# Oliverbansk/Holistic-Robot-Pose-Estimation

Measured on AMD Instinct MI355X. Metric: images/sec/GPU fwd+bwd HRNet-W32 256x256 bs=64; 1/2/4/8-GPU scaling, higher is better.
Workload: dtype bf16; 1 GPU; full network (HRNet-W32 reg backbone + HRNet-W32 DepthNet + heads + FK loss) fwd+loss+bwd+clip+Adam, BASELINE.json configs[2]; global_batch=64, per_gpu_batch=64, image=3x256x256, hrnet_w32_passes_per_image=2, parallelism=dp1, backend=single-process, rccl_ranks=1, hip_graph=True, plan_mode=hybrid, inputs=resident in HBM, optimizer=hrpe_amd.optim.FusedClipAdam (clip 5 + Adam, lr 1e-4)

## Files before the change

### holistic-robot-pose-estimation_amd/_native.py

```python
import ctypes as C
import os
import subprocess

_HERE = os.path.dirname(os.path.abspath(__file__))
LIB_PATH = os.environ.get("HRP_LIB") or os.path.join(_HERE, "libhrp_hip.so")
CSRC = os.path.join(_HERE, "csrc")

HRP_F32, HRP_BF16, HRP_F32X3 = 0, 1, 2
MAX_TAPS = 16
EW_MAX_IN = 4
EW_IDENTITY, EW_AFFINE, EW_BN_TRAIN = 0, 1, 2
FK_MAX_JOINTS, FK_MAX_KP = 32, 24
PIL_KMAX = 12


class HrpError(RuntimeError):
    pass


class ConvDesc(C.Structure):
    _fields_ = [("x", C.c_void_p), ("w", C.c_void_p), ("y", C.c_void_p), ("res", C.c_void_p),
                ("bias", C.c_void_p), ("scale", C.c_void_p), ("shift", C.c_void_p), ("stats", C.c_void_p),
                ("dtype", C.c_int32),
                ("N", C.c_int32), ("H", C.c_int32), ("W", C.c_int32), ("Cin", C.c_int32), ("x_pitch", C.c_int32),
# ... 130 lines not shown
class OptChunk(C.Structure):
    _fields_ = [("tensor", C.c_int32), ("offset", C.c_int32)]


class RegStepDesc(C.Structure):
    _fields_ = [("M", C.c_int32), ("P", C.c_int32), ("K", C.c_int32), ("N", C.c_int32),
                ("u_prev", C.c_void_p), ("u_bias", C.c_void_p), ("z", C.c_void_p), ("zw", C.c_void_p),
                ("z_len", C.c_int32), ("z_pitch", C.c_int32), ("zw_sk", C.c_int32), ("zw_sp", C.c_int32),
                ("u_out", C.c_void_p), ("a", C.c_void_p), ("a_mask", C.c_void_p), ("v", C.c_void_p),
                ("a_pitch", C.c_int32), ("v_sk", C.c_int32), ("v_sp", C.c_int32), ("a2_pitch", C.c_int32),
                ("a_out", C.c_void_p), ("w", C.c_void_p), ("bias", C.c_void_p), ("out_mask", C.c_void_p),
                ("a2", C.c_void_p), ("w2", C.c_void_p), ("w_sn", C.c_int64), ("w_sk", C.c_int64),
                ("out_pitch", C.c_int32), ("out_accumulate", C.c_int32), ("out_sum_accumulate", C.c_int32), ("w2_sk", C.c_int32),
                ("out", C.c_void_p), ("out_sum", C.c_void_p)]


class LinWgradDesc(C.Structure):
    _fields_ = [("x", C.c_void_p), ("dy", C.c_void_p), ("dw", C.c_void_p), ("dbias", C.c_void_p),
                ("x_pitch", C.c_int32), ("dy_pitch", C.c_int32), ("dw_ld", C.c_int32), ("M", C.c_int32),
                ("K", C.c_int32), ("N", C.c_int32), ("accumulate", C.c_int32), ("reserved", C.c_int32)]


REG_MAX_P, REG_MAX_PROBLEMS, LIN_WGRAD_MAX = 16, 4, 8
COPY_MAX = 16


class CopyDesc(C.Structure):
    _fields_ = [("src", C.c_void_p), ("dst", C.c_void_p), ("src_pitch", C.c_int), ("dst_pitch", C.c_int), ("rows", C.c_int),
                ("cols", C.c_int), ("accumulate", C.c_int), ("reserved", C.c_int)]


def copy_cols_batch(items, stream):
    for i0 in range(0, len(items), COPY_MAX):
        grp = items[i0:i0 + COPY_MAX]
        arr = (CopyDesc * len(grp))()
        for d, (src, sp, dst, dp, rows, cols, acc) in zip(arr, grp):
            d.src, d.src_pitch, d.dst, d.dst_pitch, d.rows, d.cols, d.accumulate = src, sp, dst, dp, rows, cols, acc
        call("hrp_copy_cols_batch", arr, len(grp), stream)


class FkChain(C.Structure):
    _fields_ = [("njoints", C.c_int32), ("parent", C.c_int32 * FK_MAX_JOINTS), ("type", C.c_int32 * FK_MAX_JOINTS),
                ("cfg", C.c_int32 * FK_MAX_JOINTS), ("mimic_mul", C.c_float * FK_MAX_JOINTS),
                ("mimic_off", C.c_float * FK_MAX_JOINTS), ("origin", (C.c_float * 12) * FK_MAX_JOINTS),
                ("axis", (C.c_float * 3) * FK_MAX_JOINTS), ("nkp", C.c_int32), ("kp_frame", C.c_int32 * FK_MAX_KP),
                ("kp_offset", (C.c_float * 3) * FK_MAX_KP), ("dof", C.c_int32)]


DREAM_BANDS = 32
DREAM_JITTER, DREAM_OCCLUSION, DREAM_SHARPNESS, DREAM_CONTRAST, DREAM_BRIGHTNESS, DREAM_COLOR = 1, 2, 4, 8, 16, 32


class DreamSample(C.Structure):
    _fields_ = [("jitter", C.c_double * 3), ("enh", C.c_double * 4), ("flags", C.c_int32),
                ("occ_x", C.c_int32), ("occ_y", C.c_int32), ("occ_w", C.c_int32), ("occ_h", C.c_int32),
                ("pad_x", C.c_int32), ("pad_y", C.c_int32), ("work_w", C.c_int32), ("work_h", C.c_int32),
                ("crop_x0", C.c_int32), ("crop_y0", C.c_int32), ("crop_x1", C.c_int32), ("crop_y1", C.c_int32),
                ("off_x", C.c_int32), ("off_y", C.c_int32), ("side", C.c_int32), ("reserved", C.c_int32),
                ("noise_off", C.c_int64), ("scratch_off", C.c_int64)]


_P, _I, _F, _L = C.c_void_p, C.c_int, C.c_float, C.c_int64
PROTOTYPES = {
    "hrp_version": [], "hrp_device_ok": [],
    "hrp_nchw_to_nhwc": [_P, _P, _I, _I, _I, _I, _I, _I, _P],
    "hrp_nhwc_to_nchw": [_P, _P, _I, _I, _I, _I, _I, _I, _P],
    "hrp_nchw_grad_from_nhwc": [_P, _P, _I, _I, _I, _I, _I, _I, _P],
    "hrp_pack_weights": [_P, _I, _I, _I, _P],
    "hrp_pack_blocks": [_I, _I, _I, _I, _I, _I],
    "hrp_pack_weights_compact": [_P, _P, _I, _I, _I, _P],
    "hrp_nchw_to_nhwc_s2d": [_P, _P, _I, _I, _I, _I, _I, _I, _P],
    "hrp_u8_nchw_to_nhwc": [_P, _P, _I, _I, _I, _I, _I, _I, _F, _I, _P],
    "hrp_gather_f32": [_P, _P, _P, _I, _I, _P],
    "hrp_pil_resize_table": [_I, _I, _P],
    "hrp_pil_resize_normalize": [_P, _I, _I, _I, _I, _P, _P, _I, _I, _P, _I, _I, _I, _P, _P, _P],
    "hrp_broadcast_hw": [_P, _I, _P, _I, _I, _I, _I, _I, _P],
    "hrp_bilinear_nhwc_to_nchw": [_P, _I, _I, _I, _I, _I, _I, _P, _I, _I, _I, _P],
    "hrp_fill_zero": [_P, _L, _P],
    "hrp_maxpool3x3s2_fwd": [_P, _I, _I, _I, _I, _I, _I, _P, _I, _P, _P],
    "hrp_maxpool3x3s2_bwd": [_P, _I, _P, _P, _I, _I, _I, _I, _I, _I, _I, _P],
    "hrp_conv2d_fwd": [C.POINTER(ConvDesc), _P],
    "hrp_conv_rowstrip_channels": [C.POINTER(ConvDesc)],
    "hrp_conv_pointwise": [C.POINTER(ConvDesc)],
    "hrp_conv2d_bwd_weight": [C.POINTER(WgradDesc), _P],
    "hrp_colsum": [_P, _I, _L, _I, _I, _P, _I, _P, _L, _P],
    "hrp_colsum_workspace_bytes": [_L, _I],
    "hrp_ew_fwd": [C.POINTER(EwDesc), _P],
    "hrp_ew_bwd_reduce": [C.POINTER(EwBwdDesc), _P],
    "hrp_ew_pool2": [_P, _I, _I, _P, _I, _I, _I, _I, _I, _P, _P],
    "hrp_ew_bwd_apply": [C.POINTER(EwBwdDesc), _P],
    "hrp_bn_running_update": [_P, _I, _P], "hrp_bn_fold": [_P, _I, _P], "hrp_bn_param_grad": [_P, _I, _P],
    "hrp_avgpool_fwd": [_P, _I, _I, _I, _I, _I, _P, _I, _P],
    "hrp_avgpool_bwd": [_P, _I, _P, _I, _I, _I, _I, _I, _I, _P],
    "hrp_softargmax3d_fwd": [_P, _I, _I, _I, _I, _I, _I, _I, _I, _I, _P, _P, _P],
    "hrp_softargmax3d_bwd": [_P, _I, _I, _I, _I, _I, _I, _I, _I, _I, _P, _P, _P, _P, _I, _P],
    "hrp_pose_geometry_fwd": [_P, _P, _P, _P, _I, _I, _I, _F, _F, _P, _P, _P, _P, _P],
    "hrp_pose_geometry_bwd": [_P, _P, _P, _P, _I, _I, _I, _F, _F, _P, _P, _P, _P, _P, _P, _P],
    "hrp_fk_project_fwd": [_P, _P, _P, _P, _P, _I, _I, _P, _P, _P, _P],
    "hrp_fk_project_bwd": [_P, _P, _P, _P, _P, _I, _I, _P, _P, _P, _P, _P, _P],
    "hrp_fk_project_rot_fwd": [_P, _P, _P, _I, _P, _P, _I, _I, _P, _P, _P, _P],
    "hrp_fk_project_rot_bwd": [_P, _P, _P, _I, _P, _P, _I, _I, _P, _P, _P, _P, _P, _P],
    "hrp_copy_cols": [_P, _I, _P, _I, _I, _I, _I, _P],
    "hrp_copy_cols_batch": [_P, _I, _P],
    "hrp_scale_rows": [_P, _I, _I, _I, _P, _F, _P],
    "hrp_mul_f32": [_P, _I, _P, _I, _P, _I, _I, _I, _I, _P],
    "hrp_opt_grad_sumsq": [_P, _P, _I, _P, _P, _P],
    "hrp_opt_adam_step": [_P, _P, _I, _P, _F, _P, _F, _F, _F, _F, _P],
    "hrp_batch_prepare": [_I, _P, _I, _P, C.POINTER(BatchInfo)],
    "hrp_batch_launch": [_P, C.POINTER(BatchInfo), _P],
    "hrp_softargmax_flat_fwd": [_P, _I, _I, _I, _I, _I, _P, _P, _P],
    "hrp_softargmax_flat_bwd": [_P, _I, _I, _I, _I, _I, _P, _P, _P, _P, _I, _P],
    "hrp_rot6d_compose_fwd": [_P, _P, _P, _I, _P],
    "hrp_rot6d_compose_bwd": [_P, _P, _P, _P, _P, _I, _I, _I, _P],
    "hrp_wgrad_fold_desc_of": [C.POINTER(WgradDesc), C.POINTER(WgradFoldDesc)],
    "hrp_batch_wgrad_fold_descs": [_P, C.POINTER(BatchInfo), C.POINTER(WgradFoldDesc)],
    "hrp_block_channels": [C.POINTER(BlockDesc)],
    "hrp_block_prepare": [_P, _I, _P, C.POINTER(BlockInfo)],
    "hrp_block_launch": [_P, C.POINTER(BlockInfo), _P],
    "hrp_pose_loss": [C.POINTER(PoseLossDesc), _P],
    "hrp_l1_loss": [_P, _P, _F, _I, _P, _P, _P],
    "hrp_sim2real_loss": [C.POINTER(Sim2RealLossDesc), _P],
    "hrp_mesh_pose": [_P, _P, _P, _P, _I, _I, _P, _P, _I, _P, _P, _P, _P],
    "hrp_mesh_pose_bwd": [_P, _P, _P, _P, _I, _I, _P, _P, _I, _P, _P, _P, _P],
    "hrp_silhouette_fwd": [C.POINTER(SilhouetteDesc), _P],
    "hrp_silhouette_bwd": [C.POINTER(SilhouetteDesc), _P, _P, _P],
    "hrp_linear_fwd": [_P, _I, _P, _P, _P, _I, _P, _I, _I, _I, _I, _P, _L, _P],
    "hrp_linear_bwd_data": [_P, _I, _P, _P, _I, _I, _I, _I, _I, _P, _L, _P],
    "hrp_linear_workspace_bytes": [_I, _I, _I],
    "hrp_linear_bwd_weight": [_P, _I, _P, _I, _P, _P, _I, _I, _I, _I, _P],
    "hrp_rng_advance": [_P, _P],
    "hrp_dropout_f32": [_P, _I, _P, _I, _P, _I, _I, _F, _P, C.c_uint32, _P],
    "hrp_dropout_masks": [_P, _L, _F, _P, C.c_uint32, _P],
    "hrp_regressor_step": [_P, _I, _P],
    "hrp_linear_wgrad_batch": [_P, _I, _P],
    "hrp_project_fwd": [_P, _P, _I, _I, _P, _P],
    "hrp_project_bwd": [_P, _P, _P, _I, _I, _P, _P],
    "hrp_pnp_solve": [_P, _P, _I, _P, _I, _P, _I, _I, _P, _P, _P, _P],
    "hrp_pnp_bwd": [_P, _P, _I, _P, _I, _P, _P, _I, _I, _I, _P, _P, _P, _P, _P, _P, _P],
    "hrp_dream_augment": [_P, _I, _I, _I, _P, _P, _L, _I, _I, _P, _L, _P, _P],
    "hrp_dream_crop_resize": [_P, _L, _P, _P, _I, _I, _I, _P, _I, _I, _P, _I, _I, _P],
}

_lib = None


def source_hash():
    import glob
    import hashlib
    files = [os.path.basename(f) for f in glob.glob(os.path.join(CSRC, "*.hip")) + glob.glob(os.path.join(CSRC, "*.h"))]
    names = sorted(files + ["../../include/hrp.h", "Makefile"])
    h = hashlib.sha256()
    for n in names:
        with open(os.path.join(CSRC, n), "rb") as fh:
            h.update(fh.read())
    return h.hexdigest()[:16]


def build(force=False):
    if force:
        subprocess.run(["make", "-C", CSRC, "clean"], check=True, stdout=subprocess.DEVNULL)
    r = subprocess.run(["make", "-C", CSRC, "-j8"], stdout=subprocess.PIPE, stderr=subprocess.STDOUT, text=True)
    if r.returncode != 0:
        raise HrpError("building libhrp_hip.so failed:\n" + r.stdout[-4000:])
    return LIB_PATH


# ... 82 lines not shown
```

### holistic-robot-pose-estimation_amd/csrc/batch.h

```cpp
#pragma once
#include "hrp_common.h"

namespace hrp {

struct BatchHdr {
  int blk0[HRP_BATCH_MAX];
};

__device__ __forceinline__ int batch_find(const BatchHdr& h, int b, int& base) {
  int g = 0;
  base = 0;
#pragma unroll
  for (int i = 1; i < HRP_BATCH_MAX; ++i) {
    const bool ge = b >= h.blk0[i];
    g = ge ? i : g;
    base = ge ? h.blk0[i] : base;
  }
  return g;
}

static inline BatchHdr make_hdr(const int* blk0, int n) {
  BatchHdr h;
  for (int i = 0; i < HRP_BATCH_MAX; ++i) h.blk0[i] = i < n ? blk0[i] : 0x7fffffff;
  return h;
}

int conv_batch_prepare_bf16(const hrp_conv_desc* descs, int n, void* table, hrp_batch_info* info);
int conv_batch_prepare_f32(const hrp_conv_desc* descs, int n, void* table, hrp_batch_info* info);
int conv_batch_prepare_f32x3(const hrp_conv_desc* descs, int n, void* table, hrp_batch_info* info);
int conv_batch_launch_bf16(const void* table_dev, const hrp_batch_info* info, hipStream_t s);
int conv_batch_launch_f32(const void* table_dev, const hrp_batch_info* info, hipStream_t s);
int conv_batch_launch_f32x3(const void* table_dev, const hrp_batch_info* info, hipStream_t s);
int64_t conv_batch_table_bytes(int n);
int conv_check(const hrp_conv_desc* d);

int wgrad_batch_prepare(const hrp_wgrad_desc* descs, int n, void* table, hrp_batch_info* info);
int wgrad_batch_launch(const void* table_dev, const hrp_batch_info* info, hipStream_t s);
int64_t wgrad_batch_table_bytes(int n);
int wgrad_fold_prepare(const hrp_wgrad_fold_desc* descs, int n, void* table, hrp_batch_info* info);
int wgrad_fold_launch(const void* table_dev, const hrp_batch_info* info, hipStream_t s);
int64_t wgrad_fold_table_bytes(int n);

int ew_batch_prepare(int family, const void* descs, int n, void* table, hrp_batch_info* info);
int ew_batch_launch(const void* table_dev, const hrp_batch_info* info, hipStream_t s);
int64_t ew_batch_table_bytes(int family, int n);

}
```

### holistic-robot-pose-estimation_amd/csrc/conv_fwd.hip

```cpp
#include "conv_row.h"
#include "conv_pw.h"

namespace hrp {

int launch_conv_f32(const hrp_conv_desc& d, hipStream_t s);
int launch_conv_f32x3(const hrp_conv_desc& d, hipStream_t s);

int conv_check(const hrp_conv_desc* d) {
  HRP_REQUIRE(d && d->x && d->w && d->y, "conv: null pointer");
  HRP_REQUIRE(d->ntaps >= 1 && d->ntaps <= HRP_MAX_TAPS, "conv: ntaps=%d", d->ntaps);
  HRP_REQUIRE(d->dtype == HRP_F32 || d->dtype == HRP_BF16 || d->dtype == HRP_F32X3, "conv: dtype=%d", d->dtype);
  const int vec = d->dtype == HRP_BF16 ? 8 : 4;
  HRP_REQUIRE(d->Cin % vec == 0 && d->x_pitch % vec == 0 && (uintptr_t)d->x % 16 == 0,
              "conv: input channels / pitch must be multiples of %d elements (Cin=%d pitch=%d)", vec, d->Cin, d->x_pitch);
  HRP_REQUIRE((uintptr_t)d->w % 16 == 0, "conv: packed weights must be 16-byte aligned");
  HRP_REQUIRE(d->w_cout_pad % 32 == 0 && d->w_cout_pad >= d->Cout, "conv: w_cout_pad=%d Cout=%d", d->w_cout_pad, d->Cout);
  HRP_REQUIRE(d->N > 0 && d->Ho > 0 && d->Wo > 0 && d->Cout > 0 && d->Cin > 0, "conv: empty problem");
  HRP_REQUIRE(d->in_stride >= 1 && d->out_stride >= 1, "conv: strides");
  HRP_REQUIRE((d->scale == nullptr) == (d->shift == nullptr), "conv: scale and shift go together");
  PwPlan pwp;
  const bool lean_kernel = hrp_conv_rowstrip_channels(d) != 0 || pw_plan(*d, pwp) != 0;
  if (d->bnb_x && d->bnb_mask && !lean_kernel) {
    const int sz = d->dtype == HRP_BF16 ? 2 : 4;
    HRP_REQUIRE(d->stats && d->bnb_mask && d->bnb_consts, "conv: bnb_x needs stats, bnb_mask and bnb_consts");
    HRP_REQUIRE(!d->res && !d->relu && !d->bias && !d->scale, "conv: bnb_x excludes res / relu / bias / scale");
    HRP_REQUIRE(d->out_stride == 1 && d->y_H == d->Ho && d->y_W == d->Wo, "conv: bnb_x needs a launch that covers y");
    HRP_REQUIRE(d->Cout % vec == 0 && d->bnb_mask_pitch >= d->Cout / vec, "conv: bnb_x needs whole vectors (Cout=%d)", d->Cout);
    HRP_REQUIRE((uintptr_t)d->y % 16 == 0 && ((size_t)d->y_pitch * sz) % 16 == 0 && (uintptr_t)d->bnb_x % 16 == 0 &&
                ((size_t)d->bnb_x_pitch * sz) % 16 == 0 && (uintptr_t)d->bnb_consts % 16 == 0, "conv: bnb_x alignment");
  }
  if (d->pro_mode != 0 || d->pro_side || d->pro_side2 || d->pro_mask || d->res_mask)
    HRP_REQUIRE(hrp_conv_rowstrip_channels(d) != 0, "conv: pro_mode / pro_side / pro_mask / res_mask need a row-strip problem (hrp_conv_rowstrip_channels)");
  if (d->tail_mode) HRP_REQUIRE(pw_plan(*d, pwp) != 0, "conv: tail_mode needs a pointwise problem with Cin 32 / 64 and Cout %% 64 == 0 (hrp_conv_pointwise)");
  if (d->bnb_x && (!d->bnb_mask || d->res))
    HRP_REQUIRE(lean_kernel, "conv: a mask-less bnb_x / bnb_x with res needs a row-strip or pointwise problem (hrp_conv_rowstrip_channels, hrp_conv_pointwise)");
  return HRP_OK;
}

}

extern "C" int hrp_conv_rowstrip_channels(const hrp_conv_desc* d) {
  return d ? hrp::row_channels(*d) : 0;
}

extern "C" int hrp_conv_pointwise(const hrp_conv_desc* d) {
  hrp::PwPlan pw;
  return d ? hrp::pw_plan(*d, pw) : 0;
}

extern "C" int hrp_conv2d_fwd(const hrp_conv_desc* d, void* stream) {
  using namespace hrp;
  const int rc = conv_check(d);
  if (rc != HRP_OK) return rc;
  if (d->dtype == HRP_F32) return launch_conv_f32(*d, (hipStream_t)stream);
  if (d->dtype == HRP_F32X3) return launch_conv_f32x3(*d, (hipStream_t)stream);
  if (hrp_conv_rowstrip_channels(d)) return launch_conv_row(*d, (hipStream_t)stream);
  PwPlan pw;
  if (pw_plan(*d, pw)) return launch_conv_pw(*d, pw, (hipStream_t)stream);
  return launch_conv<bf16_t>(*d, (hipStream_t)stream);
}

#ifdef HRP_TIMELINE
extern "C" int hrp_debug_conv_timeline(void* dst, int nblocks, int clear) {
  if (dst) (void)hipMemcpyFromSymbol(dst, HIP_SYMBOL(hrp::g_conv_timeline), sizeof(unsigned long long) * 8 * nblocks);
  if (clear) {
    void* p = nullptr;
    (void)hipGetSymbolAddress(&p, HIP_SYMBOL(hrp::g_conv_timeline));
    (void)hipMemset(p, 0, sizeof(unsigned long long) * 8192 * 8);
  }
  return 0;
}
#endif
```

### holistic-robot-pose-estimation_amd/plan.py

```python
import collections
import contextlib
import ctypes as C
import math
import os

import torch

from . import _native as nv

BN_EPS = 1e-5
STAT_SLOTS = 8


def _rup(a, b):
    return (a + b - 1) // b * b


def _dt(dtype):
    return nv.HRP_F32 if dtype == torch.float32 else nv.HRP_BF16


def _cdt(plan, dtype):
    if dtype == torch.float32:
        return nv.HRP_F32X3 if plan.x3 else nv.HRP_F32
# ... 103 lines not shown
PLAN_MODE = os.environ.get("HRP_PLAN_MODE", "hybrid")
FUSE_BN_REDUCE = True
WGRAD_DEFER = True
WGRAD_FOLD_EVERY = 32
WGRAD_SINK = int(os.environ.get("HRP_WGRAD_SINK", "16"))
PARITY_PAD = True
ROWCONV_FUSE = True
BLOCK_END_FUSE = True
BLOCK_END_REDUCE_FUSE = True
BLOCK_FUSE = os.environ.get("HRP_BLOCK_FUSE", "1") not in ("0", "")
MASKED_RES = True
BLOCK_END_FWD_FUSE = os.environ.get("HRP_BLOCK_END_FWD", "1") not in ("0", "")
BNECK_TAIL_FUSE = os.environ.get("HRP_TAIL_FUSE", "1") not in ("0", "")
POOL_FUSE_GRADS = os.environ.get("HRP_POOL_FUSE", "0") not in ("0", "")
LAZY_INPUTS = os.environ.get("HRP_LAZY_INPUTS", "1") not in ("0", "")
ARENA_ZERO_EARLY = True
BATCHING = True
GREEDY_MERGE = True
BATCH_FAMILIES = None
PLAN_STATS = bool(os.environ.get("HRP_PLAN_STATS"))
DBG_SYNC = os.environ.get("HRP_DBG_SYNC")

MAX_TILE_DILATION = 4

PARAM_EPOCH = 0
_PLAN_SERIAL = 0


def bump_param_epoch():
    global PARAM_EPOCH
    PARAM_EPOCH += 1


Entry = collections.namedtuple("Entry", "lane path op")


class _OpList(list):

    def __init__(self, plan):
        super().__init__()
        self.plan = plan

    def append(self, op):
        list.append(self, Entry(self.plan.cur_lane, self.plan.lane_path, op))


FAMILIES = {"conv": (nv.BATCH_CONV, "hrp_conv2d_fwd", nv.ConvDesc),
            "wgrad": (nv.BATCH_WGRAD, "hrp_conv2d_bwd_weight", nv.WgradDesc),
            "ew_fwd": (nv.BATCH_EW_FWD, "hrp_ew_fwd", nv.EwDesc),
            "ew_red": (nv.BATCH_EW_BWD_REDUCE, "hrp_ew_bwd_reduce", nv.EwBwdDesc),
            "ew_app": (nv.BATCH_EW_BWD_APPLY, "hrp_ew_bwd_apply", nv.EwBwdDesc),
            "wgrad_fold": (nv.BATCH_WGRAD_FOLD, None, nv.WgradFoldDesc)}


class Launch:
    __slots__ = ("fam", "desc")

    def __init__(self, fam, desc):
        self.fam, self.desc = fam, desc

    def __call__(self, s):
        nv.call(FAMILIES[self.fam][1], C.byref(self.desc), s)

    def launches(self):
        return [self]

    def fold_desc(self):
        f = nv.WgradFoldDesc()
        nv.check(nv.lib().hrp_wgrad_fold_desc_of(C.byref(self.desc), C.byref(f)), "hrp_wgrad_fold_desc_of")
        return f

    def fold_descs(self):
        return [self.fold_desc()]

    def merge_key(self):
        d = self.desc
        if BATCH_FAMILIES is not None and self.fam not in BATCH_FAMILIES:
            return None
        esz = 2 if d.dtype == nv.HRP_BF16 else 4
        if self.fam == "conv":
            if d.ntaps not in (1, 2, 4, 9) or (d.Cin * esz) % 32 or (d.dtype != nv.HRP_BF16 and d.H == 1 and d.W == 1 and d.Cin >= 512):
                return None
            if d.ntaps == 1 and nv.lib().hrp_conv_pointwise(C.byref(d)):
                return None
            return ("conv", d.dtype, d.ntaps)
        if self.fam == "wgrad":
            return ("wgrad", d.dtype, d.ntaps, d.reserved)
        if d.C % (16 // esz):
            return None
        return (self.fam, d.dtype)

    def written(self):
        d = self.desc
        if self.fam == "conv":
            main = d.y + ((d.out_off_y * d.y_W + d.out_off_x) * d.y_pitch if d.out_stride > 1 else 0)
            return tuple(a for a in (main, d.pro_side, d.pro_side2) if a)
        if self.fam in ("wgrad", "wgrad_fold"):
            return (d.dw + 4 * d.dw_tap_off,)
        if self.fam == "ew_fwd":
            return (d.out,)
        if self.fam == "ew_red":
            return (d.sums,)
        return tuple(x for x in (d.din, d.din2) if x)


class BatchLaunch:

    def __init__(self, plan, items):
        self.plan, self.items = plan, list(items)
        self.fam = items[0].fam
        self.info, self.table, self.singles, self.folds = None, None, False, None

    def launches(self):
        return self.items

    def merge_key(self):
        return self.items[0].merge_key()

    def ws_query(self):
        n = len(self.items)
        arr = (nv.WgradDesc * n)(*[it.desc for it in self.items])
        info = nv.BatchInfo()
        nv.check(nv.lib().hrp_batch_prepare(nv.BATCH_WGRAD, arr, n, None, C.byref(info)), "hrp_batch_prepare")
        return [int(info.ws_bytes[i]) for i in range(n)]

    def prepare(self):
        famid, _, dtype = FAMILIES[self.fam]
        n = len(self.items)
        arr = (dtype * n)(*[it.desc for it in self.items])
        info = nv.BatchInfo()
        nbytes = int(nv.lib().hrp_batch_table_bytes(famid, n))
        host = (C.c_char * nbytes)()
        try:
            nv.check(nv.lib().hrp_batch_prepare(famid, arr, n, host, C.byref(info)), "hrp_batch_prepare")
        except nv.HrpError:
            if self.fam == "wgrad_fold":
                raise
            if PLAN_STATS:
                import sys
                print(f"plan: batch of {n} {self.fam} launches runs one by one ({nv.lib().hrp_last_error().decode()})", file=sys.stderr)
            self.singles = True
            return
        self.info = info
        if self.fam == "wgrad" and self.items[0].desc.phase == 1:
            folds = (nv.WgradFoldDesc * n)()
            nv.check(nv.lib().hrp_batch_wgrad_fold_descs(host, C.byref(info), folds), "hrp_batch_wgrad_fold_descs")
            self.folds = list(folds)
        self.table = torch.frombuffer(bytearray(bytes(host)), dtype=torch.uint8).to(self.plan.device)
        self.plan.keep.append(self.table)

    def fold_descs(self):
        if not self.singles:
            return self.folds
        return [it.fold_desc() for it in self.items]

    def __call__(self, s):
        if self.singles:
            for it in self.items:
                it(s)
        else:
            nv.call_batch(self, s)


class BlockLaunch:
    fam = "block"

# ... 1331 lines not shown
```

### include/hrp.h

```cpp
#ifndef HRP_H
#define HRP_H

#include <stdint.h>

#ifdef __cplusplus
extern "C" {
#endif

typedef enum { HRP_F32 = 0, HRP_BF16 = 1, HRP_F32X3 = 2 } hrp_dtype;

typedef enum {
  HRP_OK = 0,
  HRP_ERR_ARG = -1,
  HRP_ERR_LAUNCH = -2,
  HRP_ERR_NODEV = -3
} hrp_status;

#define HRP_MAX_TAPS 16

#define HRP_STAT_SLOTS 8

typedef struct hrp_conv_desc {
  const void* x;
  const void* w;
// ... 109 lines not shown
  int32_t dtype;
  int32_t N, H, W, C;
  int32_t relu;
  uint8_t* mask;
  int32_t mask_pitch;
  float* consts_out;
} hrp_ew_desc;

typedef struct hrp_ew_bwd_desc {
  const void* dout;
  const void* out;
  int32_t dout_pitch, out_pitch;
  hrp_ew_input in;
  void* din;
  int32_t din_pitch;
  double* sums;
  int32_t dtype;
  int32_t N, H, W, C;
  int32_t relu;
  int32_t accumulate;
  const uint8_t* mask;
  int32_t mask_pitch;
  void* din2;
  int32_t din2_pitch;
  int32_t accumulate2;
  const float* pooled;
} hrp_ew_bwd_desc;

typedef struct hrp_bn_entry {
  const double* stats;
  float* a;
  float* b;
  const float* c;
  const float* d;
  float* out_scale;
  float* out_shift;
  int64_t* counter;
  int32_t C;
  float count, momentum, eps;
  int32_t accumulate;
} hrp_bn_entry;

#define HRP_FK_MAX_JOINTS 32
#define HRP_FK_MAX_KP 24
typedef struct hrp_fk_chain {
  int32_t njoints;
  int32_t parent[HRP_FK_MAX_JOINTS];
  int32_t type[HRP_FK_MAX_JOINTS];
  int32_t cfg[HRP_FK_MAX_JOINTS];
  float mimic_mul[HRP_FK_MAX_JOINTS], mimic_off[HRP_FK_MAX_JOINTS];
  float origin[HRP_FK_MAX_JOINTS][12];
  float axis[HRP_FK_MAX_JOINTS][3];
  int32_t nkp;
  int32_t kp_frame[HRP_FK_MAX_KP];
  float kp_offset[HRP_FK_MAX_KP][3];
  int32_t dof;
} hrp_fk_chain;

const char* hrp_last_error(void);
int hrp_version(void);
const char* hrp_source_hash(void);
int hrp_device_ok(void);

int hrp_nchw_to_nhwc(const float* src, void* dst, int dtype, int N, int C, int H, int W, int dst_pitch, void* stream);
int hrp_nhwc_to_nchw(const void* src, float* dst, int dtype, int N, int C, int H, int W, int src_pitch, void* stream);
int hrp_nchw_grad_from_nhwc(const void* src, float* dst, int dtype, int N, int C, int H, int W, int src_pitch, void* stream);
int hrp_u8_nchw_to_nhwc(const uint8_t* src, void* dst, int dtype, int N, int C, int H, int W, int dst_pitch,
                        float divisor, int s2d, void* stream);
int hrp_pack_weights(const hrp_pack_entry* table_dev, int count, int dtype, int max_elems, void* stream);
int hrp_pack_blocks(int Cout, int Cin, int ntaps, int dtype, int has_dst, int has_dst_t);
int hrp_pack_weights_compact(const hrp_pack_entry* table_dev, const int32_t* first_block_dev, int count, int total_blocks,
                             int dtype, void* stream);
int hrp_nchw_to_nhwc_s2d(const float* src, void* dst, int dtype, int N, int C, int H, int W, int dst_pitch, void* stream);
int hrp_gather_f32(const float* src, const int32_t* idx, float* dst, int n, int accumulate, void* stream);
int hrp_fill_zero(void* p, int64_t bytes, void* stream);
int hrp_maxpool3x3s2_fwd(const void* x, int dtype, int N, int H, int W, int C, int pitch, void* y, int y_pitch,
                         uint8_t* argmax, void* stream);
int hrp_maxpool3x3s2_bwd(const void* dy, int dy_pitch, const uint8_t* argmax, void* dx, int dtype, int N, int H, int W,
                         int C, int pitch, int accumulate, void* stream);

int hrp_conv2d_fwd(const hrp_conv_desc* d, void* stream);
int hrp_conv_rowstrip_channels(const hrp_conv_desc* d);
int hrp_conv_pointwise(const hrp_conv_desc* d);
int hrp_conv2d_bwd_weight(const hrp_wgrad_desc* d, void* stream);
int64_t hrp_wgrad_workspace_bytes(const hrp_wgrad_desc* d);
int64_t hrp_colsum_workspace_bytes(int64_t rows, int C);
int hrp_colsum(const void* x, int dtype, int64_t rows, int C, int pitch, float* out, int accumulate, void* workspace,
               int64_t workspace_bytes, void* stream);

#define HRP_OPT_CHUNK 4096
typedef struct hrp_opt_tensor {
  float* param;
  float* grad;
  float* exp_avg;
  float* exp_avg_sq;
  int64_t numel;
} hrp_opt_tensor;
typedef struct hrp_opt_chunk {
  int32_t tensor;
  int32_t offset;
} hrp_opt_chunk;
int hrp_opt_grad_sumsq(const hrp_opt_tensor* tensors_dev, const hrp_opt_chunk* chunks_dev, int nchunks,
                       float* sumsq_slots, float* chunk_sums, void* stream);
int hrp_opt_adam_step(const hrp_opt_tensor* tensors_dev, const hrp_opt_chunk* chunks_dev, int nchunks,
                      const float* sumsq_slots, float max_norm, const float* step_dev,
                      float lr, float beta1, float beta2, float eps, void* stream);

int hrp_ew_fwd(const hrp_ew_desc* d, void* stream);
int hrp_ew_bwd_reduce(const hrp_ew_bwd_desc* d, void* stream);
int hrp_ew_pool2(const void* src, int src_dtype, int src_pitch, const uint8_t* mask, int mask_pitch, int N, int H, int W, int C, float* dst,
                 void* stream);
int hrp_ew_bwd_apply(const hrp_ew_bwd_desc* d, void* stream);

typedef enum {
  HRP_BATCH_CONV = 0, HRP_BATCH_WGRAD = 1, HRP_BATCH_EW_FWD = 2, HRP_BATCH_EW_BWD_REDUCE = 3, HRP_BATCH_EW_BWD_APPLY = 4,
  HRP_BATCH_WGRAD_FOLD = 5
} hrp_batch_family;
#define HRP_BATCH_MAX 32
typedef struct hrp_batch_info {
  int32_t family, n, dtype;
  int32_t variant;
  int32_t grid, lds_bytes;
  int32_t grid2;
  int32_t grid3, lds_bytes3;
  int32_t blk0[HRP_BATCH_MAX + 1];
  int32_t blk2[HRP_BATCH_MAX + 1];
  int64_t ws_bytes[HRP_BATCH_MAX];
} hrp_batch_info;
int64_t hrp_batch_table_bytes(int family, int n);
int hrp_batch_prepare(int family, const void* descs, int n, void* table_host, hrp_batch_info* info);
int hrp_batch_launch(const void* table_dev, const hrp_batch_info* info, void* stream);
int hrp_wgrad_fold_desc_of(const hrp_wgrad_desc* d, hrp_wgrad_fold_desc* out);
int hrp_batch_wgrad_fold_descs(const void* table_host, const hrp_batch_info* info, hrp_wgrad_fold_desc* out);

#define HRP_PIL_KMAX 12
int hrp_pil_resize_table(int in_size, int out_size, int32_t* out);
int hrp_pil_resize_normalize(const void* src, int src_u8, int N, int H, int W, const int32_t* xtab_dev, const int32_t* ytab_dev,
                             int Ho, int Wo, void* dst, int dtype, int dst_pitch, int s2d, const float* mean3, const float* std3,
                             void* stream);
int hrp_broadcast_hw(const float* src, int src_pitch, void* dst, int dtype, int N, int HW, int C, int dst_pitch, void* stream);
int hrp_bilinear_nhwc_to_nchw(const void* src, int dtype, int N, int h, int w, int C, int pitch, float* dst, int H, int W, int act,
                              void* stream);

#define HRP_BLOCK_MAX 2
typedef struct hrp_block_desc {
  hrp_conv_desc conv1, conv2;
} hrp_block_desc;
typedef struct hrp_block_info {
  int32_t n, grid, lds_bytes, reserved;
  int32_t first_wg[HRP_BLOCK_MAX];
  int32_t bands[HRP_BLOCK_MAX];
} hrp_block_info;
int hrp_block_channels(const hrp_block_desc* d);
int64_t hrp_block_table_bytes(void);
int hrp_block_prepare(const hrp_block_desc* descs, int n, void* table, hrp_block_info* info);
int hrp_block_launch(const void* table, const hrp_block_info* info, void* stream);

int hrp_bn_running_update(const hrp_bn_entry* table_dev, int count, void* stream);
int hrp_bn_fold(const hrp_bn_entry* table_dev, int count, void* stream);
int hrp_bn_param_grad(const hrp_bn_entry* table_dev, int count, void* stream);

int hrp_avgpool_fwd(const void* x, int dtype, int N, int HW, int C, int pitch, float* out, int out_pitch, void* stream);
int hrp_avgpool_bwd(const float* dout, int dout_pitch, void* dx, int dtype, int N, int HW, int C, int pitch, int accumulate, void* stream);

int hrp_softargmax3d_fwd(const void* logits, int dtype, int B, int J, int D, int H, int W, int pitch,
                         int root, int fix_root, float* uvd, float* ms, void* stream);
// ... 176 lines not shown
```

Measured before the change: 2026 images/sec.

## Add MFMA implicit-GEMM conv forward kernel for wide bf16 convolutions

```diff
diff --git a/holistic-robot-pose-estimation_amd/_native.py b/holistic-robot-pose-estimation_amd/_native.py
--- a/holistic-robot-pose-estimation_amd/_native.py
+++ b/holistic-robot-pose-estimation_amd/_native.py
@@ -236,6 +236,8 @@
     "hrp_conv2d_fwd": [C.POINTER(ConvDesc), _P],
     "hrp_conv_rowstrip_channels": [C.POINTER(ConvDesc)],
     "hrp_conv_pointwise": [C.POINTER(ConvDesc)],
+    "hrp_conv_gemm": [C.POINTER(ConvDesc)],
+    "hrp_conv_gemm_enable": [_I],
     "hrp_conv2d_bwd_weight": [C.POINTER(WgradDesc), _P],
     "hrp_colsum": [_P, _I, _L, _I, _I, _P, _I, _P, _L, _P],
     "hrp_colsum_workspace_bytes": [_L, _I],
diff --git a/holistic-robot-pose-estimation_amd/csrc/batch.h b/holistic-robot-pose-estimation_amd/csrc/batch.h
--- a/holistic-robot-pose-estimation_amd/csrc/batch.h
+++ b/holistic-robot-pose-estimation_amd/csrc/batch.h
@@ -33,6 +33,7 @@
 int conv_batch_launch_f32x3(const void* table_dev, const hrp_batch_info* info, hipStream_t s);
 int64_t conv_batch_table_bytes(int n);
 int conv_check(const hrp_conv_desc* d);
+int launch_conv_gemm(const hrp_conv_desc* descs, int n, hipStream_t s);
 
 int wgrad_batch_prepare(const hrp_wgrad_desc* descs, int n, void* table, hrp_batch_info* info);
 int wgrad_batch_launch(const void* table_dev, const hrp_batch_info* info, hipStream_t s);
diff --git a/holistic-robot-pose-estimation_amd/csrc/conv_fwd.hip b/holistic-robot-pose-estimation_amd/csrc/conv_fwd.hip
--- a/holistic-robot-pose-estimation_amd/csrc/conv_fwd.hip
+++ b/holistic-robot-pose-estimation_amd/csrc/conv_fwd.hip
@@ -57,6 +57,7 @@
   if (hrp_conv_rowstrip_channels(d)) return launch_conv_row(*d, (hipStream_t)stream);
   PwPlan pw;
   if (pw_plan(*d, pw)) return launch_conv_pw(*d, pw, (hipStream_t)stream);
+  if (hrp_conv_gemm(d)) return launch_conv_gemm(d, 1, (hipStream_t)stream);
   return launch_conv<bf16_t>(*d, (hipStream_t)stream);
 }
 
diff --git a/holistic-robot-pose-estimation_amd/csrc/conv_gemm.h b/holistic-robot-pose-estimation_amd/csrc/conv_gemm.h
--- /dev/null
+++ b/holistic-robot-pose-estimation_amd/csrc/conv_gemm.h
@@ -0,0 +1,263 @@
+#pragma once
+#include "conv_tile.h"
+
+namespace hrp {
+
+constexpr int GM_MAXP = 4;
+constexpr int GM_STAGE = 32768;
+constexpr int GM_OP = 128 * 2 + 16;
+constexpr int GM_LDS = 2 * GM_STAGE + 8 * 128 * 4;
+
+struct GemmProb {
+  const char* x; const char* w; char* y; const char* res;
+  const float* bias; const float* scale; const float* shift; double* stats;
+  int H, W, Ho, Wo, Cin, Cout, x_pitch;
+  int y_H, y_W, y_pitch, res_pitch, out_stride, out_off_y, out_off_x, in_stride;
+  int ntaps, w_ntaps, w_cout_pad, relu;
+  int npix, n_cout_blk, nblocks, blk0;
+  int dy[9], dx[9], wtap[9];
+};
+struct GemmArgs {
+  GemmProb p[GM_MAXP];
+  int nprob;
+};
+
+__device__ __forceinline__ void conv_gemm_body(const GemmProb& P, const int b, const int stat_slot) {
+  extern __shared__ __attribute__((aligned(16))) char smem[];
+  const int tid = threadIdx.x, lane = tid & 63;
+  const int wave = __builtin_amdgcn_readfirstlane(tid >> 6);
+  const int wc = wave & 1, wp = wave >> 1;
+  const int l31 = lane & 31, khalf = lane >> 5;
+  int bid = b;
+  if ((P.nblocks & 7) == 0) bid = (bid & 7) * (P.nblocks >> 3) + (bid >> 3);
+  const int tile = bid / P.n_cout_blk, cb = bid - tile * P.n_cout_blk;
+  const int co0 = cb * 128, pix0 = tile * 128;
+  const int HoWo = P.Ho * P.Wo;
+  const long long xps = (long long)P.x_pitch * 2;
+  const char* zero = (const char*)g_zero_page;
+  asm volatile("" : "+v"(zero));
+
+  long long xoff[4];
+  int iy0[4], ix0[4];
+#pragma unroll
+  for (int j = 0; j < 4; ++j) {
+    const int pl = (wave + 4 * j) * 8 + (lane >> 3);
+    const int pg = pix0 + pl;
+    const int c_log = (lane & 7) ^ ((pl >> 1) & 7);
+    iy0[j] = -(1 << 20); ix0[j] = 0; xoff[j] = 0;
+    if (pg < P.npix) {
+      const int n = pg / HoWo, rem = pg - n * HoWo;
+      const int oy = rem / P.Wo, ox = rem - oy * P.Wo;
+      iy0[j] = oy * P.in_stride; ix0[j] = ox * P.in_stride;
+      xoff[j] = (((long long)n * P.H + iy0[j]) * P.W + ix0[j]) * xps + c_log * 16;
+    }
+  }
+  long long wlane;
+  {
+    const int r = (wave * 64 + lane) >> 1;
+    const int h = (lane & 1) ^ ((r >> 3) & 1);
+    wlane = (long long)(co0 + r) * ROW + h * 16;
+  }
+  const long long qstride = (long long)P.w_ntaps * P.w_cout_pad * ROW;
+  const int nck = P.Cin >> 6, nst = P.ntaps * nck;
+
+  const char* px[4];
+  int xstep[4];
+  const char* pw;
+  int cur_tap = 0, cur_ck = 0;
+  auto set_tap = [&](int t) {
+    const int dy = P.dy[t], dx = P.dx[t];
+    const long long toff = ((long long)dy * P.W + dx) * xps;
+#pragma unroll
+    for (int j = 0; j < 4; ++j) {
+      const bool ok = (unsigned)(iy0[j] + dy) < (unsigned)P.H && (unsigned)(ix0[j] + dx) < (unsigned)P.W;
+      px[j] = ok ? P.x + xoff[j] + toff : zero;
+      xstep[j] = ok ? 128 : 0;
+    }
+    pw = P.w + (long long)P.wtap[t] * P.w_cout_pad * ROW + wlane;
+  };
+  auto issue = [&](int slot, char* buf) {
+    if (slot < 4) {
+      dma16(px[slot], buf + (wave + 4 * slot) * 1024);
+      px[slot] += xstep[slot];
+    } else {
+      const int q = slot - 4;
+      dma16(pw + q * qstride, buf + 16384 + q * 4096 + wave * 1024);
+    }
+  };
+  auto advance = [&]() {
+    pw += 4 * qstride;
+    if (++cur_ck == nck) {
+      cur_ck = 0;
+      if (++cur_tap < P.ntaps) set_tap(cur_tap);
+    }
+  };
+  set_tap(0);
+#pragma unroll
+  for (int s = 0; s < 8; ++s) issue(s, smem);
+  advance();
+
+  int a_off[2], b_off[2];
+#pragma unroll
+  for (int c = 0; c < 2; ++c) a_off[c] = 16384 + row_addr(wc * 64 + c * 32 + l31, khalf);
+#pragma unroll
+  for (int p = 0; p < 2; ++p) {
+    const int pix = wp * 64 + p * 32 + l31;
+    b_off[p] = pix * 128 + ((khalf ^ ((pix >> 1) & 7)) << 4);
+  }
+
+  f32x16 acc[2][2];
+#pragma unroll
+  for (int c = 0; c < 2; ++c)
+#pragma unroll
+    for (int p = 0; p < 2; ++p)
+#pragma unroll
+      for (int i = 0; i < 16; ++i) acc[c][p][i] = 0.f;
+
+  for (int st = 0; st < nst; ++st) {
+    asm volatile("s_waitcnt vmcnt(0)" ::: "memory");
+    __syncthreads();
+    const char* sb = smem + (st & 1) * GM_STAGE;
+    char* nb = smem + ((st + 1) & 1) * GM_STAGE;
+    const bool more = st + 1 < nst;
+    bf16x8 fa[2][2], fb[2][2];
+    auto load = [&](int kk, bf16x8 (&a)[2], bf16x8 (&bb)[2]) {
+#pragma unroll
+      for (int c = 0; c < 2; ++c) a[c] = *(const bf16x8*)(sb + a_off[c] + kk * 4096);
+#pragma unroll
+      for (int p = 0; p < 2; ++p) bb[p] = *(const bf16x8*)(sb + (b_off[p] ^ (kk * 32)));
+    };
+    load(0, fa[0], fb[0]);
+#pragma unroll
+    for (int kk = 0; kk < 4; ++kk) {
+      const int cur = kk & 1, nxt = cur ^ 1;
+      if (kk + 1 < 4) load(kk + 1, fa[nxt], fb[nxt]);
+#pragma unroll
+      for (int c = 0; c < 2; ++c)
+#pragma unroll
+        for (int p = 0; p < 2; ++p)
+          acc[c][p] = __builtin_amdgcn_mfma_f32_32x32x16_bf16(fa[cur][c], fb[cur][p], acc[c][p], 0, 0, 0);
+      if (more) {
+        issue(2 * kk, nb);
+        issue(2 * kk + 1, nb);
+      }
+      __builtin_amdgcn_sched_barrier(0);
+    }
+    if (more) advance();
+  }
+  __syncthreads();
+
+  char* lds_out = smem;
+  float* lds_stats = (float*)(smem + 2 * GM_STAGE);
+#pragma unroll
+  for (int c = 0; c < 2; ++c) {
+#pragma unroll
+    for (int q4 = 0; q4 < 4; ++q4) {
+      const int cl = wc * 64 + c * 32 + 8 * q4 + 4 * khalf;
+      float bia[4] = {0.f, 0.f, 0.f, 0.f}, sc[4] = {1.f, 1.f, 1.f, 1.f}, sh[4] = {0.f, 0.f, 0.f, 0.f};
+      if (P.bias || P.scale) {
+#pragma unroll
+        for (int i = 0; i < 4; ++i) {
+          const int co = co0 + cl + i;
+          if (P.bias) bia[i] = P.bias[co];
+          if (P.scale) { sc[i] = P.scale[co]; sh[i] = P.shift[co]; }
+        }
+      }
+#pragma unroll
+      for (int p = 0; p < 2; ++p) {
+        const int m = wp * 64 + p * 32 + l31;
+        float v[4];
+#pragma unroll
+        for (int i = 0; i < 4; ++i) v[i] = acc[c][p][4 * q4 + i];
+        if (P.bias || P.scale) {
+#pragma unroll
+          for (int i = 0; i < 4; ++i) v[i] = (v[i] + bia[i]) * sc[i] + sh[i];
+        }
+        uint2 r;
+        r.x = pack_bf2(v[0], v[1]);
+        r.y = pack_bf2(v[2], v[3]);
+        *(uint2*)(lds_out + m * GM_OP + cl * 2) = r;
+      }
+    }
+  }
+  __syncthreads();
+
+  float s1[8], s2[8];
+#pragma unroll
+  for (int i = 0; i < 8; ++i) s1[i] = s2[i] = 0.f;
+  const int cv = tid & 15;
+  const int co = co0 + cv * 8;
+#pragma unroll
+  for (int k = 0; k < 8; ++k) {
+    const int m = (tid >> 4) + k * 16;
+    const int pg = pix0 + m;
+    if (pg >= P.npix) continue;
+    const int n = pg / HoWo, rem = pg - n * HoWo;
+    const int oy = rem / P.Wo, ox = rem - oy * P.Wo;
+    const size_t opix = ((size_t)n * P.y_H + (oy * P.out_stride + P.out_off_y)) * P.y_W + (ox * P.out_stride + P.out_off_x);
+    const uint4 raw = *(const uint4*)(lds_out + m * GM_OP + cv * 16);
+    float f[8];
+    Elem<bf16_t>::unpack(raw, f);
+    if (!P.res && !P.relu) {
+      *(uint4*)(P.y + (opix * P.y_pitch + co) * 2) = raw;
+      if (P.stats) {
+#pragma unroll
+        for (int i = 0; i < 8; ++i) { s1[i] += f[i]; s2[i] += f[i] * f[i]; }
+      }
+    } else {
+      if (P.res) {
+        float r[8];
+        Elem<bf16_t>::unpack(*(const uint4*)(P.res + (opix * P.res_pitch + co) * 2), r);
+#pragma unroll
+        for (int i = 0; i < 8; ++i) f[i] += r[i];
+      }
+      if (P.relu) {
+#pragma unroll
+        for (int i = 0; i < 8; ++i) f[i] = fmaxf(f[i], 0.f);
+      }
+      const uint4 packed = Elem<bf16_t>::pack(f);
+      *(uint4*)(P.y + (opix * P.y_pitch + co) * 2) = packed;
+      if (P.stats) {
+        float g[8];
+        Elem<bf16_t>::unpack(packed, g);
+#pragma unroll
+        for (int i = 0; i < 8; ++i) { s1[i] += g[i]; s2[i] += g[i] * g[i]; }
+      }
+    }
+  }
+  if (P.stats) {
+#pragma unroll
+    for (int i = 0; i < 8; ++i) {
+#pragma unroll
+      for (int o = 32; o >= 16; o >>= 1) {
+        s1[i] += __shfl_xor(s1[i], o, 64);
+        s2[i] += __shfl_xor(s2[i], o, 64);
+      }
+    }
+    if (lane < 16) {
+#pragma unroll
+      for (int i = 0; i < 8; ++i) {
+        lds_stats[(wave * 2 + 0) * 128 + lane * 8 + i] = s1[i];
+        lds_stats[(wave * 2 + 1) * 128 + lane * 8 + i] = s2[i];
+      }
+    }
+    __syncthreads();
+    const int which = tid >> 7, ch = tid & 127;
+    const float v = lds_stats[(0 * 2 + which) * 128 + ch] + lds_stats[(1 * 2 + which) * 128 + ch] +
+                    lds_stats[(2 * 2 + which) * 128 + ch] + lds_stats[(3 * 2 + which) * 128 + ch];
+    double* slot = P.stats + (size_t)stat_slot * 2 * P.Cout;
+    atomicAdd(&slot[which * P.Cout + co0 + ch], (double)v);
+  }
+}
+
+__global__ __launch_bounds__(256, 2) void conv_gemm_kernel(const GemmArgs a) {
+  int pi = 0;
+  for (int i = 1; i < a.nprob; ++i)
+    if ((int)blockIdx.x >= a.p[i].blk0) pi = i;
+  pi = __builtin_amdgcn_readfirstlane(pi);
+  const GemmProb& P = a.p[pi];
+  if ((int)blockIdx.x - P.blk0 >= P.nblocks) return;
+  conv_gemm_body(P, blockIdx.x - P.blk0, blockIdx.x & (HRP_STAT_SLOTS - 1));
+}
+
+}
diff --git a/holistic-robot-pose-estimation_amd/csrc/conv_gemm.hip b/holistic-robot-pose-estimation_amd/csrc/conv_gemm.hip
--- /dev/null
+++ b/holistic-robot-pose-estimation_amd/csrc/conv_gemm.hip
@@ -0,0 +1,82 @@
+#include "conv_gemm.h"
+
+namespace hrp {
+
+static int g_gemm_on = -1;
+static int gemm_on() {
+  if (g_gemm_on < 0) {
+    const char* e = getenv("HRP_CONV_GEMM");
+    g_gemm_on = (e && e[0] == '0' && e[1] == 0) ? 0 : 1;
+  }
+  return g_gemm_on;
+}
+
+static inline int gemm_blocks(const hrp_conv_desc& d) {
+  const long npix = (long)d.N * d.Ho * d.Wo;
+  return (int)((npix + 127) / 128) * (d.Cout / 128);
+}
+
+static bool gemm_shape_ok(const hrp_conv_desc& d) {
+  if (d.dtype != HRP_BF16) return false;
+  if (d.Cin < 128 || d.Cin % 64 || d.Cout < 128 || d.Cout % 128) return false;
+  if (d.ntaps != 1 && d.ntaps != 2 && d.ntaps != 4 && d.ntaps != 9) return false;
+  if (d.pro_mode || d.pro_side || d.pro_side2 || d.pro_mask || d.res_mask || d.tail_mode || d.bnb_x) return false;
+  if (d.N < 1 || d.Ho < 1 || d.Wo < 1 || d.in_stride < 1 || d.out_stride < 1) return false;
+  if ((long)d.N * d.Ho * d.Wo >= (1L << 30)) return false;
+  if (d.x_pitch % 8 || d.x_pitch < d.Cin || d.y_pitch % 8 || d.y_pitch < d.Cout || (uintptr_t)d.x % 16 || (uintptr_t)d.y % 16) return false;
+  if (d.res && (d.res_pitch % 8 || (uintptr_t)d.res % 16)) return false;
+  if (d.w_cout_pad < d.Cout) return false;
+  for (int i = 0; i < d.ntaps; ++i)
+    if (d.wtap[i] < 0 || d.wtap[i] >= d.w_ntaps) return false;
+  return true;
+}
+
+static bool gemm_fill_ok(int blocks) { return blocks >= 256 || blocks <= 16; }
+
+static void gemm_fill(const hrp_conv_desc& d, GemmProb& P, int blk0) {
+  P.x = (const char*)d.x; P.w = (const char*)d.w; P.y = (char*)d.y; P.res = (const char*)d.res;
+  P.bias = d.bias; P.scale = d.scale; P.shift = d.shift; P.stats = d.stats;
+  P.H = d.H; P.W = d.W; P.Ho = d.Ho; P.Wo = d.Wo; P.Cin = d.Cin; P.Cout = d.Cout; P.x_pitch = d.x_pitch;
+  P.y_H = d.y_H; P.y_W = d.y_W; P.y_pitch = d.y_pitch; P.res_pitch = d.res_pitch;
+  P.out_stride = d.out_stride; P.out_off_y = d.out_off_y; P.out_off_x = d.out_off_x; P.in_stride = d.in_stride;
+  P.ntaps = d.ntaps; P.w_ntaps = d.w_ntaps; P.w_cout_pad = d.w_cout_pad; P.relu = d.relu;
+  P.npix = d.N * d.Ho * d.Wo;
+  P.n_cout_blk = d.Cout / 128;
+  P.nblocks = gemm_blocks(d);
+  P.blk0 = blk0;
+  for (int i = 0; i < 9; ++i) {
+    P.dy[i] = i < d.ntaps ? d.dy[i] : 0; P.dx[i] = i < d.ntaps ? d.dx[i] : 0; P.wtap[i] = i < d.ntaps ? d.wtap[i] : 0;
+  }
+}
+
+int launch_conv_gemm(const hrp_conv_desc* descs, int n, hipStream_t s) {
+  GemmArgs a = {};
+  int blocks = 0;
+  for (int i = 0; i < n; ++i) {
+    gemm_fill(descs[i], a.p[i], blocks);
+    blocks += (a.p[i].nblocks + 7) & ~7;
+  }
+  a.nprob = n;
+  static bool attr_set = false;
+  if (!attr_set) {
+    (void)hipFuncSetAttribute((const void*)conv_gemm_kernel, hipFuncAttributeMaxDynamicSharedMemorySize, GM_LDS);
+    attr_set = true;
+  }
+  hipLaunchKernelGGL(conv_gemm_kernel, dim3(blocks), dim3(256), GM_LDS, s, a);
+  return check_launch("conv_gemm_kernel");
+}
+
+}
+
+extern "C" int hrp_conv_gemm(const hrp_conv_desc* d) {
+  using namespace hrp;
+  if (!d || !gemm_on() || !gemm_shape_ok(*d)) return 0;
+  if (hrp_conv_rowstrip_channels(d) || hrp_conv_pointwise(d)) return 0;
+  return gemm_fill_ok(gemm_blocks(*d)) ? 1 : 0;
+}
+
+extern "C" int hrp_conv_gemm_enable(int on) {
+  const int was = hrp::gemm_on();
+  if (on >= 0) hrp::g_gemm_on = on ? 1 : 0;
+  return was;
+}
diff --git a/holistic-robot-pose-estimation_amd/plan.py b/holistic-robot-pose-estimation_amd/plan.py
--- a/holistic-robot-pose-estimation_amd/plan.py
+++ b/holistic-robot-pose-estimation_amd/plan.py
@@ -209,6 +209,8 @@
             if d.ntaps not in (1, 2, 4, 9) or (d.Cin * esz) % 32 or (d.dtype != nv.HRP_BF16 and d.H == 1 and d.W == 1 and d.Cin >= 512):
                 return None
             if d.ntaps == 1 and nv.lib().hrp_conv_pointwise(C.byref(d)):
+                return None
+            if nv.lib().hrp_conv_gemm(C.byref(d)):
                 return None
             return ("conv", d.dtype, d.ntaps)
         if self.fam == "wgrad":
diff --git a/include/hrp.h b/include/hrp.h
--- a/include/hrp.h
+++ b/include/hrp.h
@@ -215,6 +215,8 @@
 int hrp_conv2d_fwd(const hrp_conv_desc* d, void* stream);
 int hrp_conv_rowstrip_channels(const hrp_conv_desc* d);
 int hrp_conv_pointwise(const hrp_conv_desc* d);
+int hrp_conv_gemm(const hrp_conv_desc* d);
+int hrp_conv_gemm_enable(int on);
 int hrp_conv2d_bwd_weight(const hrp_wgrad_desc* d, void* stream);
 int64_t hrp_wgrad_workspace_bytes(const hrp_wgrad_desc* d);
 int64_t hrp_colsum_workspace_bytes(int64_t rows, int C);
```

Result: no change. 2042 images/sec (median of 6 runs) (+0.8%).
